# Yongda1/Ab-initio-Flexible-Gaussian-Basis-Neural-Network-Quantum-Monte-Carlo

Hardware: AMD Instinct MI355X
Metric: walker·steps/sec + local-energy evals/sec, N2 14e⁻ 4096 walkers, 1/2/4/8 MI355X (higher is better)
Workload: dtype f32

## Files before the change

ab-initio-flexible-gaussian-basis-neural-network-quantum-monte-carlo_amd/csrc/walker_rev.h:

```cpp
#pragma once
#include "jets.h"
#include "layout.h"
#include "kargs.h"
#include "limdrift.h"
#include "gj.h"
#include "electron.h"

namespace aq {

#ifdef AQ_PHASE_PROF
static __device__ unsigned long long aq_phase_cycles[32];
#define AQ_PH(k)                                                                         \
  do {                                                                                   \
    const unsigned long long t_ = __builtin_readcyclecounter();                          \
    if (lane == 0) atomicAdd(&aq_phase_cycles[(ka.proposal ? 16 : 0) + (k)], t_ - t_ph); \
    t_ph = t_;                                                                           \
  } while (0)
#elif defined(AQ_PHASE_MARK)
#define AQ_PH(k) asm volatile(";AQMARK " #k)
#elif defined(AQ_STOP_AFTER)
#define AQ_PH(k)                                                                     \
  do {                                                                               \
    if constexpr (PROP && (k) == AQ_STOP_AFTER) {                                    \
      if (ka.logabs) ((T*)ka.logabs)[conf * 64 + lane] = sm[lane] + sm[lane + 1024]; \
      return;                                                                        \
    }                                                                                \
  } while (0)
#else
#define AQ_PH(k) \
  do {           \
  } while (0)
#endif

#ifdef AQ_ABLATE
#define AQ_ABL(b) (isprop && (ka.ablate & (b)))
#else
#define AQ_ABL(b) false
#endif

template <typename T> __device__ __forceinline__ T pt_rec(T t) {
  return T(0.70710678118654752) * (T(1) - t * t);
}
template <typename T, int N, int A, bool FWDREG = false>
struct SmemRev {
  static constexpr int D0 = 4 * A;
  static constexpr int DFM = 3 * D0 + 8;
  static constexpr int QM = DFM / 4;
  static constexpr int hl_n = N * D0 + N * 4;
  static constexpr int cmax(int a, int b) { return a > b ? a : b; }
  static constexpr int xs = 0;
  static constexpr int hl = 48;
  static constexpr int hbar = hl;
  static constexpr int QL = (3 * 4 + 8) / 4;
  static constexpr int cq = hl + hl_n;
  static constexpr int sv = cq + (FWDREG ? 0 : N * QM + 2 * N * QL);
  static constexpr int cqo(int l, int i) { return l == 0 ? i * QM : N * QM + ((l - 1) * N + i) * QL; }
  static constexpr int g2 = sv + (FWDREG ? 0 : 3 * N * 4);
  static constexpr int yv = g2 + 3 * 2 * N * 4;
  static constexpr int ybar = yv;
  static constexpr int R = yv + N * N;
  static constexpr int ph = R;
  static constexpr int mx = R + N * N * 2;
  static constexpr int dbar = R;
  static constexpr int R_n = cmax(cmax(4 * N * N, 3 * N * N), 4 + 64 * 12);
  static constexpr int pv = g2;
  static constexpr int RW = (N + 3) / 4;
  static constexpr int st = ((g2 + 3 * N + 2 + 3) / 4) * 4;
  static constexpr int zr = st + (4 * RW * 4 * 4 + (int)sizeof(T) - 1) / (int)sizeof(T);
  static_assert(zr + 4 <= g2 + 3 * 2 * N * 4, "slot table outside the g2 region");
  static constexpr int jdo = R + R_n;
  static constexpr bool hand = FWDREG;
  static constexpr int th = (jdo + (FWDREG ? 64 : 0) + 3) / 4 * 4;
  static constexpr int end = hand ? th + 2 * 2 * 16 * 4 : jdo + (FWDREG ? 64 : 0);
  static constexpr int bytes = ((end * (int)sizeof(T)) + 15) & ~15;
  static constexpr int hoff(int l) { return l == 0 ? 0 : N * D0; }
};

template <int N, int A>
struct WCache {
  static constexpr int D0 = 4 * A;
  static constexpr int yv = 0;
  static constexpr int h0 = yv + N * N;
  static constexpr int loc = h0 + N * D0;
  static constexpr int jaev = loc + (N + D0) * 48;
  static constexpr int jaed = jaev + N;
  static constexpr int g2 = jaed + 48;
  static constexpr int jee = g2 + 3 * 2 * N * 4;
  static constexpr int pv = jee + 1;
  static constexpr int pt = ((pv + 3 * N + 2 + 3) / 4) * 4;
  static constexpr int size = ((pt + 8 * N * N + 63) / 64) * 64;
};
template <int N, int A>
struct ECache {
  static constexpr int D0 = 4 * A;
  static constexpr int yv = 0;
  static constexpr int h0 = N;
  static constexpr int yd = N + D0;
  static constexpr int hd = yd + 3 * N;
  static constexpr int jv = hd + 3 * D0;
  static constexpr int jd = jv + 1;
  static constexpr int xp = jd + 3;
  static constexpr int size = ((xp + 3 + 15) / 16) * 16;
};

template <typename T, int N, int A>
__device__ __forceinline__ void pair_values(const T d[3], cptr<T> P, T out[3][4], T tq[2][4]) {
  using Ly = Lay<N, A>;
  const T RSQ2 = T(0.70710678118654752);
  T p[4];
  p[0] = f_sqrt(d[0] * d[0] + d[1] * d[1] + d[2] * d[2]);
#pragma unroll
  for (int c = 0; c < 3; ++c) p[1 + c] = d[c];
#pragma unroll
  for (int f = 0; f < 4; ++f) out[0][f] = p[f];
#pragma unroll
  for (int j = 0; j < 2; ++j) {
    const cptr<T> dw = P + (j == 0 ? Ly::dbl_w0 : Ly::dbl_w1);
    const cptr<T> db = P + (j == 0 ? Ly::dbl_b0 : Ly::dbl_b1);
    T q[4];
#pragma unroll
    for (int o = 0; o < 4; ++o) {
      T s = db[o];
#pragma unroll
      for (int m = 0; m < 4; ++m) s += p[m] * dw[m * 4 + o];
      q[o] = f_tanh(s);
    }
#pragma unroll
    for (int o = 0; o < 4; ++o) {
      tq[j][o] = q[o];
      p[o] = (p[o] + q[o]) * RSQ2;
      out[j + 1][o] = p[o];
    }
  }
}
template <typename T, int N, int A>
__device__ __forceinline__ void pair_values(const T d[3], cptr<T> P, T out[3][4]) {
  T tq[2][4];
  pair_values<T, N, A>(d, P, out, tq);
}

template <typename T> __device__ __forceinline__ T class4_sum(T x) {
  x += dpp<0x124>(x);
  x += dpp<0x128>(x);
  x += __shfl_xor(x, 16);
  x += __shfl_xor(x, 32);
  return x;
}
template <int M, typename T> __device__ __forceinline__ T quad_bcast(T x) {
  return dpp<M | (M << 2) | (M << 4) | (M << 6)>(x);
}

template <typename T, int NV, int NU>
__device__ __forceinline__ void ld_use(cptr<T> p, T* out) {
  static_assert(NU <= NV, "record");
  if constexpr (sizeof(T) == 4) {
    typedef float f4 __attribute__((ext_vector_type(4)));
// ... 276 lines not shown
    }
#pragma unroll
    for (int o = 0; o < 4; ++o) p1[o] = (p0[o] + f1[o]) * RSQ2;
#pragma unroll
    for (int o = 0; o < 4; ++o) {
      T s = Pq[Ly::dbl_b1 + o];
#pragma unroll
      for (int m = 0; m < 4; ++m) s += p1[m] * Pq[Ly::dbl_w1 + m * 4 + o];
      f2[o] = f_tanh(s);
    }
#pragma unroll
    for (int o = 0; o < 4; ++o) {
      t1[o] = fresh ? pt_rec(f1[o]) : t1[o];
      t2[o] = fresh ? pt_rec(f2[o]) : t2[o];
    }
  }
  T pb2[4], pb1[4], pb0[4];
#pragma unroll
  for (int f = 0; f < 4; ++f) pb2[f] = g2b[((2 * 2 + G) * N + i) * 4 + f];
  T z2[4];
#pragma unroll
  for (int o = 0; o < 4; ++o) z2[o] = pb2[o] * t2[o];
#pragma unroll
  for (int m = 0; m < 4; ++m) {
    T s = g2b[((1 * 2 + G) * N + i) * 4 + m] + pb2[m] * RSQ2;
#pragma unroll
    for (int o = 0; o < 4; ++o) s += z2[o] * Pq[Ly::dbl_w1 + m * 4 + o];
    pb1[m] = s;
  }
  T z1[4];
#pragma unroll
  for (int o = 0; o < 4; ++o) z1[o] = pb1[o] * t1[o];
#pragma unroll
  for (int m = 0; m < 4; ++m) {
    T s = g2b[((0 * 2 + G) * N + i) * 4 + m] + pb1[m] * RSQ2;
#pragma unroll
    for (int o = 0; o < 4; ++o) s += z1[o] * Pq[Ly::dbl_w0 + m * 4 + o];
    pb0[m] = s;
  }
  T rb = pb0[0];
  {
    const T den = al * r + T(1);
    rb += and_zero(k < i, cusp * f_rcp(den * den));
  }
  const T ir = f_rcp(r);
#pragma unroll
  for (int c = 0; c < 3; ++c) dbar[(k * N + i) * 3 + c] = pb0[1 + c] + rb * d[c] * ir;
}

template <typename T, int N>
__device__ __forceinline__ void walker_draws(const __attribute__((address_space(4))) KArgs* kl, int conf, int lane) {
  if (kl->dg1 && lane < N) {
    const uint32_t t = (uint32_t)(conf * N + lane);
    const uint64_t seed = kl->seed, step = kl->step;
    float a[3], b[3], c[4];
    philox_normal3f(seed, step, t, 0u, a);
    philox_normal3f(seed, step, t, 1u, b);
    philox_u4(seed, step, t, 2u, c);
#pragma unroll
    for (int k = 0; k < 3; ++k) {
      ((T*)kl->dg1)[(size_t)t * 3 + k] = (T)a[k];
      ((T*)kl->dg2)[(size_t)t * 3 + k] = (T)b[k];
    }
    ((T*)kl->du)[t] = (T)(c[0] - 5.9604644775390625e-08f);
  }
}

template <typename T, int N, int A, bool PREP = false, bool PROP = false, bool PH = false, bool SPL = false>
__global__ __attribute__((amdgpu_flat_work_group_size(1, 64 * (SPL ? 2 : RevWpb<T, PROP, PREP>::value)))) __attribute__((amdgpu_waves_per_eu(RevWaves<T, N, A, PREP, PROP>::value))) void
k_walker_rev(KArgs ka) {
  static_assert(!PH || PREP, "PH is an adjoint-pass instantiation");
  static_assert(!SPL || (!PROP && !PREP), "SPL is a walker-launch instantiation");
  using Ly = Lay<N, A>;
  constexpr bool fwd_reg = PROP;
  constexpr bool xlane = PROP;
  using SM = SmemRev<T, N, A, fwd_reg>;
  using LCc = LapCache<N, A>;
  static_assert(URecordFits<Ly::total_ext>::value && URecordFits<WCache<N, A>::size>::value &&
                    URecordFits<ECache<N, A>::size>::value && URecordFits<LCc::size>::value &&
                    URecordFits<3 * N>::value && sizeof(PairTab<N>) < (1u << 28),
                "record too large for a 32-bit lane offset");
  constexpr int D0 = SM::D0;
  constexpr int WPB = SPL ? 2 : RevWpb<T, PROP, PREP>::value;
  const cptr<T> P = param_ptr<T>(ka.prm);
  extern __shared__ __attribute__((aligned(16))) unsigned char smem_raw[];
  const int wv = WPB > 1 ? __builtin_amdgcn_readfirstlane((int)(threadIdx.x >> 6)) : 0;
  T* sm = (T*)(smem_raw + (SPL ? 0 : wv) * SM::bytes);
  T* xs = sm + SM::xs;

  const bool isprop = PROP ? true : (ka.proposal != 0);
  const int conf = SPL ? xcd_major(blockIdx.x, gridDim.x) : xcd_major(blockIdx.x, gridDim.x) * WPB + wv;
  if (WPB > 1 && conf >= ka.nconf) return;
  const int lane = WPB > 1 ? (int)(threadIdx.x & 63) : (int)threadIdx.x;
  const int lc = lane >> 4;
  const int er = lane & 15;
  const int le = er < N ? er : N - 1;
  const bool val = (lc == 3);
  const bool live = er < N;
  const bool dir = (lc < 3) && live;
  const int nup = ka.nup;
  const T tstep = (T)ka.tstep;
  const T RSQ2 = T(0.70710678118654752);
  const T ginv0 = T(1) / T(nup), ginv1 = T(1) / T(N - nup);
  const int* rowsrc = ka.rowsrc;
#ifdef AQ_PHASE_PROF
  unsigned long long t_ph = __builtin_readcyclecounter();
#endif

  int pb = conf, pi = -1;
  if (isprop) {
    const int mper = ka.mper ? ka.mper : N, mdiv = ka.mdiv ? ka.mdiv : 1;
    pb = conf / mper;
    pi = (conf - pb * mper) / mdiv;
  }
  const T te_walk = (!PROP && isprop && !ka.xnew) ? taueff_wave<T>(ka.taueff, ka.tacc, 0, ka.tstep, ka.tpart) : T(0);
  if (SPL && wv != 0) {
  } else if (!PREP && !isprop && ka.acc.lpn) {
    const T te1 = taueff_wave<T>(ka.acc.taueff, ka.acc.tacc, 0, ka.acc.tstep, ka.acc.tpart);
    const T te2 = taueff_wave<T>(ka.acc.taueff, ka.acc.tacc, 1, ka.acc.tstep, ka.acc.tpart);
    if (lane < N) {
      T xn[3];
      const bool acc = accept_one<T, N>(ka.acc, (const T*)ka.pos, conf, lane, xn, te1, te2);
#pragma unroll
      for (int c = 0; c < 3; ++c) xs[3 * lane + c] = xn[c];
      if (acc) {
#pragma unroll
        for (int c = 0; c < 3; ++c) ((T*)ka.pos)[(size_t)conf * 3 * N + 3 * lane + c] = xn[c];
        if (ka.acc.count) atomicAdd(&ka.acc.count[conf], 1);
      }
    }
  } else if (!PROP && lane < 3 * N) {
    T x = ((const T*)ka.pos)[(size_t)pb * 3 * N + lane];
    if (isprop && lane / 3 == pi) {
      sm[SM::R + (lane - 3 * pi)] = x;
      if (ka.xnew) {
        x = ((const T*)ka.xnew)[(size_t)conf * 3 + (lane - 3 * pi)];
      } else {
        const T z = ((const T*)ka.gauss1)[(size_t)pb * 3 * N + lane];
        const T ge = ((const T*)ka.pgrad)[(size_t)pb * 3 * N + lane] * te_walk;
        x = x + (ge * tstep + f_sqrt(tstep) * z);
      }
    }
    xs[lane] = x;
  }
  if constexpr (SPL) __syncthreads();
  else if constexpr (!PROP) AQ_SYNC();

  AQ_PH(0);
  using WC = WCache<N, A>;
  using EC = ECache<N, A>;
  const bool reuse = !PREP && PROP;
  const bool wfix = !PREP && !PROP && !isprop && ka.pvok != 0;
  T* Wc = (T*)ka.wcache + (size_t)(reuse ? pb : conf) * WC::size;
  if constexpr (PROP) Wc = ubase(Wc);
  T* Lw = PREP ? (T*)ka.lapcache + (size_t)conf * LCc::size : nullptr;
  const T* Eq = reuse ? (const T*)ka.ecache + (size_t)conf * EC::size : nullptr;
  T* Yv = sm + SM::yv;
  T* g2 = sm + SM::g2;
  T jv = T(0), jd1 = T(0), jve = T(0);
  T jsum_p = T(0);
  T pvr = T(0);
  int rsl = 0;
  T jvp = T(0);
  auto f2_pair_values = [&](T cusp, T al) {
    T* S = sm + SM::R + 4;
    const T* xo = sm + SM::R;
    const int o = lane & 15, part = lane >> 4;
    const int os = o < N ? o : N - 1;
    const T* xp = (part & 1) ? xo : xs + pi * 3;
    T d[3];
#pragma unroll
    for (int c = 0; c < 3; ++c) d[c] = (part < 2) ? xs[os * 3 + c] - xp[c] : xp[c] - xs[os * 3 + c];
    T v[3][4], tq[2][4];
    pair_values<T, N, A>(d, P, v, tq);
    if constexpr (SM::hand) {
      if ((part & 1) == 0 && o < N && o != pi) {
#pragma unroll
        for (int j = 0; j < 2; ++j) {
          T* th = (T*)__builtin_assume_aligned(sm + SM::th + (((part >> 1) * 2 + j) * 16 + o) * 4, 16);
#pragma unroll
          for (int f = 0; f < 4; ++f) th[f] = pt_rec(tq[j][f]);
        }
      }
    }
#pragma unroll
    for (int l = 0; l < 3; ++l)
#pragma unroll
      for (int f = 0; f < 4; ++f) S[lane * 12 + l * 4 + f] = v[l][f];
    if (part < 2 && o < N && o != pi) {
      if constexpr (!PROP) {
        cusp = P[Ly::jee_c + pi * N + o];
        al = P[Ly::jee_a + pi * N + o];
      }
      const T je = f_div(cusp * v[0][0], al * v[0][0] + T(1));
      jvp += part == 0 ? je : -je;
    }
  };
  auto jee_params = [&](T& cusp, T& al) {
    const int os = (lane & 15) < N ? (lane & 15) : N - 1;
    const cptr<T> row = P + pi * N;
    cusp = *uat(row + Ly::jee_c, (unsigned)os);
    al = *uat(row + Ly::jee_a, (unsigned)os);
  };
  if (reuse) {
    lds_dma<T, N * N>(Yv, Wc + WC::yv, lane);
    lds_dma<T, N * D0>(sm + SM::hl, Wc + WC::h0, lane);
    lds_dma<T, 3 * 2 * N * 4>(g2, Wc + WC::g2, lane);
    const T eyv = *uat(Eq + EC::yv, (unsigned)(lane < N ? lane : N - 1));
    const T eh0 = *uat(Eq + EC::h0, (unsigned)(lane < D0 ? lane : D0 - 1));
    const bool mvl = lane < 3 * N && lane / 3 == pi;
    T x0 = T(0), xm = T(0), jc = T(0), ja = T(0);
    if constexpr (PROP) {
      const int l3 = lane < 3 * N ? lane : 3 * N - 1;
      x0 = *uat((const T*)ka.pos + (size_t)pb * 3 * N, (unsigned)l3);
      xm = *uat(Eq + EC::xp, (unsigned)(mvl ? lane - 3 * pi : 0));
      jee_params(jc, ja);
      rsl = *uat(rowsrc, (unsigned)(lane < N ? lane : N - 1));
    }
    {
      if constexpr (PROP) {
        const T* js = (er == pi) ? Eq + EC::jv : Wc + WC::jaev + le;
        jv = and_zero(val && live, *js);
        const T* ds = (le == pi) ? Eq + EC::jd + (lc < 3 ? lc : 0) : Wc + WC::jaed + (lane < 48 ? lane : 47);
        jd1 = and_zero(dir, *ds);
        jve = and_zero(lane == 0, Wc[WC::jee]);
      } else {
        const T a = Wc[WC::jaev + le], b = Eq[EC::jv];
        jv = (val && live) ? ((er == pi) ? b : a) : T(0);
        const T a1 = Wc[WC::jaed + (lane < 48 ? lane : 47)], b1 = Eq[EC::jd + (lc < 3 ? lc : 0)];
        jd1 = dir ? ((le == pi) ? b1 : a1) : T(0);
        const T a2 = Wc[WC::jee];
        jve = lane == 0 ? a2 : T(0);
      }
      pvr = *uat(Wc + WC::pv, (unsigned)(lane < 2 * N + 2 ? lane : 2 * N + 1));
    }
    if constexpr (PROP) {
      if (mvl) sm[SM::R + (lane - 3 * pi)] = x0;
      if (lane < 3 * N) xs[lane] = mvl ? xm : x0;
      AQ_SYNC();
      f2_pair_values(jc, ja);
    }
    asm volatile("s_waitcnt vmcnt(0)" ::: "memory");
    if (lane < N) Yv[pi * N + lane] = eyv;
    if (lane < D0) sm[SM::hl + pi * D0 + lane] = eh0;
  } else if (!SPL || wv == 0) {
    if (wfix) pvr = Wc[WC::pv + (lane < 3 * N + 2 ? lane : 3 * N + 1)];
    ElecOut<T, A> eo;
    electron_stage<T, N, A>(P, xs + le * 3, le, lc, eo);
    T* Wl = Wc + WC::loc + lane;
#pragma unroll
    for (int col = 0; col < N; ++col) {
      PJ<T> sy = P[Ly::wy + col] * eo.yst[0];
#pragma unroll
      for (int m = 1; m < NYW; ++m) sy = sy + P[Ly::wy + m * N + col] * eo.yst[m];
      const PJ<T> yt = eo.env * sy;
      if (!PREP && lane < 48) Wl[col * 48] = yt.d1;
      if (val && live) Yv[er * N + col] = yt.v;
    }
#pragma unroll
    for (int m = 0; m < D0; ++m) {
      if (!PREP && lane < 48) Wl[(N + m) * 48] = eo.hf[m].d1;
      if (val && live) sm[SM::hl + er * D0 + m] = eo.hf[m].v;
    }
    jv = (val && live) ? eo.jae.v : T(0);
    jd1 = dir ? eo.jae.d1 : T(0);
    if (!PREP && !isprop) {
      if (val && live) Wc[WC::jaev + er] = eo.jae.v;
      if (lane < 48) Wc[WC::jaed + lane] = jd1;
    }
  }
  AQ_SYNC();
  if (!PREP && !isprop && (!SPL || wv == 0)) {
    for (int idx = lane; idx < N * N; idx += 64) Wc[WC::yv + idx] = Yv[idx];
    for (int idx = lane; idx < N * D0; idx += 64) Wc[WC::h0 + idx] = sm[SM::hl + idx];
  }

  AQ_PH(1);
  if (reuse && !AQ_ABL(1)) {
    T* S = sm + SM::R + 4;
    if constexpr (!PROP) {
      f2_pair_values(T(0), T(0));
      AQ_SYNC();
    }
    jve += jvp;
    if constexpr (fwd_reg) {
      jsum_p = wave_sum(jv + jve);
      sm[SM::jdo + lane] = jd1;
      jv = jve = jd1 = T(0);
    }
    if (lane < 16) {
      if (lane < N && lane != pi) {
        const int Gp = pi >= nup ? 1 : 0;
        const T gw = Gp ? ginv1 : ginv0;
#pragma unroll
        for (int l = 0; l < 3; ++l)
#pragma unroll
          for (int f = 0; f < 4; ++f)
            g2[((l * 2 + Gp) * N + lane) * 4 + f] +=
                (S[lane * 12 + l * 4 + f] - S[(16 + lane) * 12 + l * 4 + f]) * gw;
      }
    } else if (lane < 40) {
      const int t = lane - 16;
      const int l = t >> 3, G = (t >> 2) & 1, f = t & 3;
      const int k0 = G ? nup : 0, k1 = G ? N : nup;
      T acc = T(0);
#pragma unroll
      for (int k = 0; k < N; ++k) {
        const T dv = S[(32 + k) * 12 + l * 4 + f] - S[(48 + k) * 12 + l * 4 + f];
        acc += (k >= k0 && k < k1 && k != pi) ? dv : T(0);
      }
      g2[((l * 2 + G) * N + pi) * 4 + f] += acc * (G ? ginv1 : ginv0);
    }
  } else if (!reuse && (!SPL || wv == 1)) {
    {
      const int i = lane >> 2, kq = lane & 3;
      const bool icol = i < N;
      const int ii = icol ? i : N - 1;
      T acc[3][2][4];
  #pragma unroll
      for (int l = 0; l < 3; ++l)
  #pragma unroll
        for (int G = 0; G < 2; ++G)
  #pragma unroll
          for (int f = 0; f < 4; ++f) acc[l][G][f] = T(0);
      constexpr int NT = (N + 3) / 4;
      T jcp[NT], jap[NT];
  #pragma unroll
      for (int t = 0; t < NT; ++t) {
        const int kk = kq + 4 * t < N ? kq + 4 * t : N - 1;
        jcp[t] = P[Ly::jee_c + kk * N + ii];
        jap[t] = P[Ly::jee_a + kk * N + ii];
      }
      T dwv[2][16], dbv[2][4];
  #pragma unroll
      for (int j = 0; j < 2; ++j) {
        const cptr<T> dw = P + (j == 0 ? Ly::dbl_w0 : Ly::dbl_w1);
        const cptr<T> db = P + (j == 0 ? Ly::dbl_b0 : Ly::dbl_b1);
  #pragma unroll
        for (int k = 0; k < 16; ++k) dwv[j][k] = dw[k];
  #pragma unroll
        for (int k = 0; k < 4; ++k) dbv[j][k] = db[k];
      }
  #pragma unroll
      for (int t = 0; t < NT; ++t) {
        const int k = kq + 4 * t;
        if (k < N) {
          const bool diag = (k == ii);
          T d[3];
  #pragma unroll
          for (int c = 0; c < 3; ++c) d[c] = xs[ii * 3 + c] - xs[k * 3 + c];
          const T r2 = d[0] * d[0] + d[1] * d[1] + d[2] * d[2];
          const T r = f_sqrt(diag ? T(1) : r2);
          T p[4] = {diag ? T(0) : r, diag ? T(0) : d[0], diag ? T(0) : d[1], diag ? T(0) : d[2]};
          if (icol && k < ii) {
            const T cusp = jcp[t], al = jap[t];
            jve += f_div(cusp * r, al * r + T(1));
          }
          const bool G1 = k >= nup;
  #pragma unroll
          for (int f = 0; f < 4; ++f) {
            acc[0][0][f] += G1 ? T(0) : p[f];
            acc[0][1][f] += G1 ? p[f] : T(0);
          }
  #pragma unroll
          for (int j = 0; j < 2; ++j) {
            T q[4];
  #pragma unroll
            for (int o = 0; o < 4; ++o) {
              T s = dbv[j][o];
  #pragma unroll
              for (int m = 0; m < 4; ++m) s += p[m] * dwv[j][m * 4 + o];
              q[o] = f_tanh(s);
            }
            if (!PREP && !isprop && icol && !diag) {
              T* tp = Wc + WC::pt + (k * N + ii) * 8 + j * 4;
#pragma unroll
              for (int o = 0; o < 4; ++o) tp[o] = pt_rec(q[o]);
            }
            if (PREP && icol) {
              T* tp = Lw + LCc::pt + (k * N + ii) * LCc::pt_n + j * 4;
#pragma unroll
              for (int o = 0; o < 4; ++o) tp[o] = q[o];
            }
  #pragma unroll
            for (int o = 0; o < 4; ++o) {
              p[o] = (p[o] + q[o]) * RSQ2;
              acc[j + 1][0][o] += G1 ? T(0) : p[o];
              acc[j + 1][1][o] += G1 ? p[o] : T(0);
            }
          }
        }
// ... 134 lines not shown
  for (int l = 0; l < 3; ++l) {
    const int d1 = l == 0 ? D0 : NH;
    const int DF = 3 * d1 + 8;
    const int Q = DF / 4;
    const int T4 = d1 / 4;
    if (l + 1 < 3) lw_load(l + 1);
    if constexpr (PROP) {
      if (l == 2) orb_load();
    }
    asm volatile("" ::: "memory");
    T hown[D0 / 4];
    if (l == 0) {
#pragma unroll
      for (int t = 0; t < D0 / 4; ++t) hown[t] = hl[ic * D0 + ff + 4 * t];
    } else {
#pragma unroll
      for (int t = 0; t < D0 / 4; ++t) hown[t] = hreg;
    }
    T gown[2][D0 / 4];
#pragma unroll
    for (int t = 0; t < D0 / 4; ++t) {
      if (t < T4) {
        const T x = ilive ? hown[t] : T(0);
        gown[0][t] = class4_sum(inG1 ? T(0) : x) * ginv0;
        gown[1][t] = class4_sum(inG1 ? x : T(0)) * ginv1;
      }
    }
    T zc[SM::QM];
#pragma unroll
    for (int q = 0; q < SM::QM; ++q) {
      if (q < Q) {
        T F;
        if (q < T4) F = hown[q];
        else if (q < 3 * T4) F = gown[(q - T4) / T4][(q - T4) % T4];
        else F = g2[((l * 2 + (q - 3 * T4)) * N + ic) * 4 + ff];
        T z = F * wcv[l][q];
        asm volatile("" : "+v"(z));
        z += dpp<0xB1>(z);
        z += dpp<0x4E>(z);
        zc[q] = z;
      }
    }
    const int QF = Q / 4;
    T cq[SM::QM];
#pragma unroll
    for (int s4 = 0; s4 < SM::QM / 4; ++s4) {
      if (s4 < QF) {
        const int q0 = 4 * s4;
        T z0 = zc[q0], z1 = zc[q0 + 1], z2 = zc[q0 + 2], z3 = zc[q0 + 3];
        asm volatile("" : "+v"(z0), "+v"(z1), "+v"(z2), "+v"(z3));
        const T zs = (ff & 2) ? ((ff & 1) ? z3 : z2) : ((ff & 1) ? z1 : z0);
        const T c = f_tanh(zs * T(0.25) + wcb[l][s4]);
        if constexpr (fwd_reg) cqr[l][s4] = c;
        else if (ilive) cqv[SM::cqo(l, ic) + q0 + ff] = c;
        cq[q0 + 0] = quad_bcast<0>(c);
        cq[q0 + 1] = quad_bcast<1>(c);
        cq[q0 + 2] = quad_bcast<2>(c);
        cq[q0 + 3] = quad_bcast<3>(c);
      }
    }
#pragma unroll
    for (int q = 0; q < SM::QM; ++q) {
      if (q >= 4 * QF && q < Q) {
        cq[q] = f_tanh(zc[q] * T(0.25) + wcb[l][q]);
        if constexpr (fwd_reg) cqr[l][QF + q - 4 * QF] = cq[q];
        else if (ilive && (q & 3) == ff) cqv[SM::cqo(l, ic) + q] = cq[q];
      }
    }
    T z = wsb[l], z1 = T(0);
#pragma unroll
    for (int q = 0; q < SM::QM; ++q)
      if (q < Q) {
        if (q & 1) z1 += cq[q] * wsw[l][q];
        else z += cq[q] * wsw[l][q];
      }
    z += z1;
    const T sval = f_tanh(z);
    if constexpr (fwd_reg) svr[l] = sval;
    else if (ilive) sv[(l * N + ic) * 4 + ff] = sval;
    const T hin = l == 0 ? hl[ic * D0 + ff] : hreg;
    hreg = (d1 == NH) ? (hin + sval) * RSQ2 : sval;
  }
  }
  if (ilive) hl[SM::hoff(3) + ic * 4 + ff] = hreg;
  AQ_SYNC();
  if ((reuse || wfix) && lane < (wfix ? 3 * N + 2 : 2 * N + 2)) sm[SM::pv + lane] = pvr;
  if constexpr (PROP) {
    const int r = (int)pvr;
    const int src = __shfl(rsl, lane < N ? r : 0);
    if (lane < 4 * SM::RW) {
      const bool ok = lane < N;
      const bool up = r < nup;
      const int h = SM::hl + SM::hoff(3) + src * 4;
      int* stab = (int*)(sm + SM::st) + 4 * lane;
      stab[0] = ok ? SM::yv + r * N : SM::yv;
      stab[1] = (ok && up) ? h : SM::zr;
      stab[2] = (ok && !up) ? h : SM::zr;
      stab[3] = ok ? (up ? 0 : 1) : 2;
    }
    if (lane < 4) sm[SM::zr + lane] = T(0);
    AQ_SYNC();
  }

  AQ_PH(3);
  T* Ph = sm + SM::ph;
  T* Mx = sm + SM::mx;
  const T* H3 = hl + SM::hoff(3);
  for (int idx = PROP ? N * N : lane; idx < N * N; idx += 64) {
    const int r = idx / N, col = idx - r * N;
    const int src = rowsrc[r];
    const int sp = r < nup ? 0 : 1;
    T re = T(0), im = T(0);
#pragma unroll
    for (int f = 0; f < 4; ++f) {
      const T hv = H3[src * 4 + f];
      re += hv * P[Ly::orb_w + ((sp * 4 + f) * N + col) * 2 + 0];
      im += hv * P[Ly::orb_w + ((sp * 4 + f) * N + col) * 2 + 1];
    }
    re += P[Ly::orb_b + (sp * N + col) * 2 + 0];
    im += P[Ly::orb_b + (sp * N + col) * 2 + 1];
    Ph[idx * 2 + 0] = re;
    Ph[idx * 2 + 1] = im;
  }
  if constexpr (!PROP) AQ_SYNC();
  T logdet, phr, phi;
  constexpr bool ybar_reg = PROP;
  V2o a2[(N + 3) / 4];
  if (reuse) {
    bool bad = false;
    logdet = phr = phi = T(0);
    if constexpr (PROP) {
      constexpr int RW = (N + 3) / 4;
      using V2 = typename Pair<T>::type;
      const int cc = lane & 15, rg = lane >> 4;
      const T* rec = sm + SM::pv;
      const int ccl = cc < N ? cc : N - 1;
      const V2* w = ow;
      const V2* bsp = obs;
      const int* stab = (const int*)(sm + SM::st) + 4 * RW * rg;
      if constexpr (phi_mfma) {
        typedef float v4f __attribute__((ext_vector_type(4)));
        const int* sti = (const int*)(sm + SM::st) + 4 * (lane & 15);
        const int fq = lane >> 4;
        const float hu = sm[sti[1] + fq], hd = sm[sti[2] + fq];
        int yo4[RW], fl4[RW];
        v4f pre, pim;
#pragma unroll
        for (int t = 0; t < RW; ++t) {
          yo4[t] = stab[4 * t];
          fl4[t] = stab[4 * t + 3];
          pre[t] = fl4[t] == 1 ? pair_re<T>(bsp[1]) : pair_re<T>(bsp[0]);
          pim[t] = fl4[t] == 1 ? pair_im<T>(bsp[1]) : pair_im<T>(bsp[0]);
        }
        pre = __builtin_amdgcn_mfma_f32_16x16x4f32(hu, owm[0], pre, 0, 0, 0);
        pim = __builtin_amdgcn_mfma_f32_16x16x4f32(hu, owm[1], pim, 0, 0, 0);
        pre = __builtin_amdgcn_mfma_f32_16x16x4f32(hd, owm[2], pre, 0, 0, 0);
        pim = __builtin_amdgcn_mfma_f32_16x16x4f32(hd, owm[3], pim, 0, 0, 0);
#pragma unroll
        for (int t = 0; t < RW; ++t) {
          const bool ok = fl4[t] != 2 && cc < N;
          if (ok) {
            const int e = yo4[t] - SM::yv + cc;
            Ph[e * 2 + 0] = pre[t];
            Ph[e * 2 + 1] = pim[t];
          }
          const T y = ok ? sm[yo4[t] + ccl] : T(0);
          a2[t] = pair_make<T>(pre[t] * y, pim[t] * y);
        }
      } else
#pragma unroll
      for (int t = 0; t < RW; ++t) {
        const int yo = stab[4 * t], hu = stab[4 * t + 1], hd = stab[4 * t + 2], fl = stab[4 * t + 3];
        V2 acc = fl == 1 ? bsp[1] : bsp[0];
#pragma unroll
        for (int f = 0; f < 4; ++f) acc = pair_fma<T>(sm[hu + f], w[f], acc);
#pragma unroll
        for (int f = 0; f < 4; ++f) acc = pair_fma<T>(sm[hd + f], w[4 + f], acc);
        const bool ok = fl != 2 && cc < N;
        if (ok) {
          const int e = yo - SM::yv + cc;
          Ph[e * 2 + 0] = pair_re<T>(acc);
          Ph[e * 2 + 1] = pair_im<T>(acc);
        }
        const T y = ok ? sm[yo + ccl] : T(0);
        a2[t] = pair_make<T>(pair_re<T>(acc) * y, pair_im<T>(acc) * y);
      }
      __builtin_amdgcn_s_setprio(1);
      if (!AQ_ABL(4)) gj_fixed_regs<T, N>(a2, Mx, lane, rec, logdet, phr, phi, bad);
      __builtin_amdgcn_s_setprio(0);
    } else
    if (!AQ_ABL(4)) gj_inverse_fixed<T, N>(Ph, Yv, Mx, lane, sm + SM::pv, logdet, phr, phi, bad);
#ifdef AQ_ABLATE
    if (ka.ablate) bad = false;
#endif
    if (bad) {
#ifdef AQ_PHASE_PROF
      if (lane == 0) atomicAdd(&aq_phase_cycles[15], 1ull);
#endif
#ifdef AQ_PHASE_MARK
      AQ_PH(10);
#endif
      gj_inverse<T, N>(Ph, Yv, Mx, lane, logdet, phr, phi);
      if constexpr (ybar_reg) {
        wave_sync();
        const int cc = lane & 15, rg = lane >> 4;
        const int r = (int)sm[SM::pv + (cc < N ? cc : 0)];
#pragma unroll
        for (int t = 0; t < (N + 3) / 4; ++t) {
          const int c = rg * ((N + 3) / 4) + t;
          const int e = ((c < N ? c : 0) * N + r) * 2;
          a2[t] = pair_make<T>(Mx[e], Mx[e + 1]);
        }
      }
#ifdef AQ_PHASE_MARK
      AQ_PH(11);
#endif
    }
  } else {
    bool bad = true;
    if (wfix) gj_inverse_fixed<T, N>(Ph, Yv, Mx, lane, sm + SM::pv, logdet, phr, phi, bad, Wc + WC::pv, 2 * N + 2);
    if (bad) gj_inverse<T, N>(Ph, Yv, Mx, lane, logdet, phr, phi, (!PREP && !isprop) ? Wc + WC::pv : nullptr);
  }
  if constexpr (!PREP) {
    if (ka.value_only) {
      const T jsum = fwd_reg ? jsum_p : wave_sum(jv + jve);
      const T lpsi = logdet + jsum;
      if (lane == 0) {
        if (ka.logabs) ((T*)ka.logabs)[conf] = lpsi;
        if (ka.phase) ((T*)ka.phase)[conf] = f_atan2(phi, phr);
      }
      if (ka.orb) {
        const T je = wave_sum(jve), ja = wave_sum(jv);
        const T sc = f_exp(je / T(N)) * f_exp(ja / T(N));
        T* O = (T*)ka.orb + (size_t)conf * N * N * 2;
        for (int idx = lane; idx < N * N; idx += 64) {
          const T y = Yv[idx] * sc;
          O[2 * idx] = Ph[2 * idx] * y;
          O[2 * idx + 1] = Ph[2 * idx + 1] * y;
        }
      }
      return;
    }
  }
  AQ_SYNC();
#define BRE(c, s) Mx[((c) * N + (s)) * 2]
#define BIM(c, s) Mx[((c) * N + (s)) * 2 + 1]

  AQ_PH(4);
  T* hbar = sm + SM::hbar;
  T* ybar = sm + SM::ybar;
  constexpr bool q_mfma = PREP && sizeof(T) == 4 && NH == 4;
  if (!q_mfma && lane < 4 * N && !AQ_ABL(8)) {
    const int r = lane >> 2, f = lane & 3;
    const int sp = r < nup ? 0 : 1;
    const cptr<T> wrow = uat(ubase(P + Ly::orb_w), (unsigned)((sp * 4 + f) * N * 2));
    T q = T(0), q1 = T(0);
#pragma unroll
    for (int c = 0; c < N; ++c) {
      const T yv = Yv[r * N + c];
      const T wr = wrow[c * 2] * yv;
      const T wi = wrow[c * 2 + 1] * yv;
      const T qc = PH ? wr * BIM(c, r) + wi * BRE(c, r) : wr * BRE(c, r) - wi * BIM(c, r);
      if (c & 1) q1 += qc;
      else q += qc;
    }
    q += q1;
    hbar[SM::hoff(3) + *uat(rowsrc, (unsigned)r) * 4 + f] = q;
  }
  if constexpr (PREP) {
    for (int idx = lane; idx < 2 * N * N; idx += 64) {
      Lw[LCc::bm + idx] = Mx[idx];
      Lw[LCc::ph + idx] = Ph[idx];
    }
    if constexpr (q_mfma) {
      typedef float v4f __attribute__((ext_vector_type(4)));
      constexpr int NM = (4 * N + 15) / 16, NK = (N + 3) / 4;
      const int kq = lane >> 4, e = lane & 15, fq = lane & 3;
      float bre[NK], bim[NK], wr[2][NK], wi[2][NK];
#pragma unroll
      for (int kk = 0; kk < NK; ++kk) {
        const int c = 4 * kk + kq;
        const bool bok = c < N && e < N;
        const int cl = c < N ? c : N - 1, el = e < N ? e : N - 1;
        bre[kk] = bok ? (float)BRE(cl, el) : 0.f;
        bim[kk] = bok ? (float)BIM(cl, el) : 0.f;
#pragma unroll
        for (int sp = 0; sp < 2; ++sp) {
          const float a = P[Ly::orb_w + ((sp * 4 + fq) * N + cl) * 2], b = P[Ly::orb_w + ((sp * 4 + fq) * N + cl) * 2 + 1];
          wr[sp][kk] = c < N ? a : 0.f;
          wi[sp][kk] = c < N ? b : 0.f;
        }
      }
#pragma unroll
      for (int m = 0; m < NM; ++m) {
        const int r = 4 * m + (e >> 2);
        const bool rok = r < N;
        const bool up = r < nup;
        v4f qre = {0.f, 0.f, 0.f, 0.f}, qim = {0.f, 0.f, 0.f, 0.f};
#pragma unroll
        for (int kk = 0; kk < NK; ++kk) {
          const int c = 4 * kk + kq;
          const float y = (rok && c < N) ? (float)Yv[(rok ? r : 0) * N + (c < N ? c : 0)] : 0.f;
          const float ur = (up ? wr[0][kk] : wr[1][kk]) * y, ui = (up ? wi[0][kk] : wi[1][kk]) * y;
          qre = __builtin_amdgcn_mfma_f32_16x16x4f32(ur, bre[kk], qre, 0, 0, 0);
          qre = __builtin_amdgcn_mfma_f32_16x16x4f32(-ui, bim[kk], qre, 0, 0, 0);
          qim = __builtin_amdgcn_mfma_f32_16x16x4f32(ur, bim[kk], qim, 0, 0, 0);
          qim = __builtin_amdgcn_mfma_f32_16x16x4f32(ui, bre[kk], qim, 0, 0, 0);
        }
// ... 217 lines not shown
            const T* gl = gb + (j + 1) * 2 * N * 4;
            T tv[4];
#pragma unroll
            for (int o = 0; o < 4; ++o) tv[o] = tcur[j * 4 + o];
#pragma unroll
            for (int c = 0; c < NC; ++c) {
              T z1[4], z2[4];
#pragma unroll
              for (int o = 0; o < 4; ++o) {
                T a1 = T(0), a2 = (j == 0) ? p2[c][0] * dw[o] : T(0);
#pragma unroll
                for (int mm = 0; mm < 4; ++mm) {
                  a1 += p1[c][mm] * dw[mm * 4 + o];
                  if (j > 0) a2 += p2[c][mm] * dw[mm * 4 + o];
                }
                z1[o] = a1;
                z2[o] = a2;
              }
#pragma unroll
              for (int o = 0; o < 4; ++o) {
                const T sd1 = T(1) - tv[o] * tv[o];
                const T t1 = sd1 * z1[o];
                const T t2 = sd1 * (z2[o] - T(2) * tv[o] * z1[o] * z1[o]);
                p1[c][o] = (p1[c][o] + t1) * RSQ2;
                p2[c][o] = (p2[c][o] + t2) * RSQ2;
                s1[j][c][o] += m * p1[c][o];
                pcurv += m * gl[o] * p2[c][o];
              }
            }
          }
        }
#pragma unroll
        for (int c = 0; c < NC; ++c) {
          s0[c] += dpp<0xB1>(s0[c]);
          s0[c] += dpp<0x4E>(s0[c]);
#pragma unroll
          for (int j = 0; j < 2; ++j)
#pragma unroll
            for (int f = 0; f < 4; ++f) {
              s1[j][c][f] += dpp<0xB1>(s1[j][c][f]);
              s1[j][c][f] += dpp<0x4E>(s1[j][c][f]);
            }
        }
        if (ilv && kq < NC) {
          const int c = C0 + kq;
          const T cnt = T(k1 - k0 - ((ii >= k0 && ii < k1) ? 1 : 0));
          T* o0 = Lw + LCc::sd + ((G * N + ii) * 3 + c) * 4;
          o0[0] = (NC == 1 || kq == 0) ? s0[0] : s0[NC - 1];
#pragma unroll
          for (int f = 1; f < 4; ++f) o0[f] = (f - 1 == c) ? cnt : T(0);
#pragma unroll
          for (int j = 0; j < 2; ++j) {
            T* oj = Lw + (j + 1) * LCc::layer_n + LCc::sd + ((G * N + ii) * 3 + c) * 4;
#pragma unroll
            for (int f = 0; f < 4; ++f) oj[f] = (NC == 1 || kq == 0) ? s1[j][0][f] : s1[j][NC - 1][f];
          }
        }
      }
    };
    pair_pass(std::integral_constant<int, 0>{}, std::integral_constant<int, 2>{});
    pair_pass(std::integral_constant<int, 2>{}, std::integral_constant<int, 1>{});
    pcurv = T(2) * wave_sum(pcurv);
    const T lpsi = logdet + wave_sum(jv + jve);
    if (lane == 0) {
      Lw[LCc::scal] = pcurv;
      if (ka.logabs) ((T*)ka.logabs)[conf] = lpsi;
      if (ka.phase) ((T*)ka.phase)[conf] = f_atan2(phi, phr);
    }
    return;
  }

  const int c4 = lc < 3 ? lc : 0;
  T lv[N + D0];
  auto lv_load = [&]() {
    const bool mov = reuse && le == pi;
    const T* la = mov ? Eq + EC::yd + c4 * N : Wc + WC::loc + (lane < 48 ? lane : 47);
    const T* lb = mov ? Eq + EC::hd + c4 * D0 : Wc + WC::loc + N * 48 + (lane < 48 ? lane : 47);
    const int st = mov ? 1 : 48;
#pragma unroll
    for (int m = 0; m < N; ++m) lv[m] = la[m * st];
#pragma unroll
    for (int m = 0; m < D0; ++m) lv[N + m] = lb[m * st];
  };
  lv_load();
  AQ_PH(6);
  T* dbar = sm + SM::dbar;
  auto pair_adjoint = [&](int k, int i, bool may_fresh, bool fresh, const T* tcache, T cusp, T al) {
    b3_pair_adjoint<T, N, A>(P, xs, g2b, dbar, nup, k, i, may_fresh, fresh, tcache, cusp, al);
  };
  constexpr int NPR = N * (N - 1);
  if (reuse && !AQ_ABL(32)) {
    constexpr int M = 2 * (N - 1);
    constexpr int NIT = (NPR + 63) / 64;
    T tc[NIT][8], jc[NIT], ja[NIT];
    int pk[NIT], pi2[NIT];
    unsigned prow[NIT];
#pragma unroll
    for (int u = 0; u < NIT; ++u) {
      const unsigned code = uat(&pair_tab<N>.v[pi][0], (unsigned)lane)[64 * u];
      const int k = code & 15, i = (code >> 4) & 15;
      pk[u] = k;
      pi2[u] = i;
      prow[u] = code >> 8;
      jc[u] = *uat(P + Ly::jee_c, prow[u]);
      ja[u] = *uat(P + Ly::jee_a, prow[u]);
    }
#pragma unroll
    for (int u = 0; u < NIT; ++u) {
      const T* tp = uat(Wc + WC::pt, prow[u] * 8);
#pragma unroll
      for (int o = 0; o < 8; ++o) tc[u][o] = tp[o];
    }
    if constexpr (SM::hand) {
      const int hp = pk[0] == pi ? 0 : 1, ho = pk[0] == pi ? pi2[0] : pk[0];
      T hv[8];
#pragma unroll
      for (int j = 0; j < 2; ++j) {
        const T* th = (const T*)__builtin_assume_aligned(sm + SM::th + ((hp * 2 + j) * 16 + ho) * 4, 16);
#pragma unroll
        for (int f = 0; f < 4; ++f) hv[j * 4 + f] = th[f];
      }
#pragma unroll
      for (int o = 0; o < 8; ++o) tc[0][o] = lane < M ? hv[o] : tc[0][o];
    }
#pragma unroll
    for (int u = 0; u < NIT; ++u) {
      const int it = lane + 64 * u;
      if (it < NPR) pair_adjoint(pk[u], pi2[u], false, false, tc[u], jc[u], ja[u]);
    }
  } else if (!reuse) {
    if (!PREP && !isprop && ka.wcache) {
      if constexpr (SPL) __syncthreads();
      __builtin_amdgcn_fence(__ATOMIC_RELEASE, "workgroup");
      __builtin_amdgcn_fence(__ATOMIC_ACQUIRE, "workgroup");
      for (int it = lane; it < NPR; it += SPL ? 128 : 64) {
        const int k = it / (N - 1);
        const int jj = it - k * (N - 1);
        const int i = jj + (jj >= k ? 1 : 0);
        pair_adjoint(k, i, false, false, Wc + WC::pt + (k * N + i) * 8, P[Ly::jee_c + k * N + i], P[Ly::jee_a + k * N + i]);
      }
      if constexpr (SPL) __syncthreads();
    } else {
      for (int it = lane; it < NPR; it += 64) {
        const int k = it / (N - 1);
        const int jj = it - k * (N - 1);
        const int i = jj + (jj >= k ? 1 : 0);
        pair_adjoint(k, i, true, true, nullptr, P[Ly::jee_c + k * N + i], P[Ly::jee_a + k * N + i]);
      }
    }
  }
  AQ_SYNC();

  AQ_PH(7);
  T g = fwd_reg ? sm[SM::jdo + lane] : jd1;
  if (!AQ_ABL(64)) {
    T ga = T(0), gb = T(0), gc = T(0);
#pragma unroll
    for (int k = 0; k < N; ++k) {
      const T dk = dbar[(k * N + le) * 3 + c4] - dbar[(le * N + k) * 3 + c4];
      if (k & 1) ga += (k == le) ? T(0) : dk;
      else g += (k == le) ? T(0) : dk;
    }
#pragma unroll
    for (int col = 0; col < N; ++col) {
      if (col & 1) gc = f_fma(ybar[le * N + col], lv[col], gc);
      else gb = f_fma(ybar[le * N + col], lv[col], gb);
    }
#pragma unroll
    for (int m = 0; m < D0; ++m) {
      if (m & 1) gc = f_fma(hbar[le * D0 + m], lv[N + m], gc);
      else gb = f_fma(hbar[le * D0 + m], lv[N + m], gb);
    }
    g = (g + ga) + (gb + gc);
  }

  AQ_PH(8);
  const T gd = dir ? g : T(0);
  const T sumsq = wave_sum(gd * gd);
  const T lpsi = logdet + (fwd_reg ? jsum_p : wave_sum(jv + jve));
  const auto* kl = late_args();
  if (kl->grad && dir) *uat((T*)kl->grad + (size_t)conf * 3 * N, (unsigned)(3 * le + lc)) = g;
  if (kl->gown && dir && le == pi) *uat((T*)kl->gown + (size_t)conf * 3, (unsigned)lc) = g;
  if (lane == 0) {
    if (kl->logabs) ((T*)kl->logabs)[conf] = lpsi;
    if (kl->phase) ((T*)kl->phase)[conf] = f_atan2(phi, phr);
    if (kl->sumsq) ((T*)kl->sumsq)[conf] = sumsq;
    if (kl->tacc) tacc_add(kl->tacc, isprop ? 1 : 0, conf, (double)sumsq);
  }
  if constexpr (!PREP && !SPL) {
    if (!isprop) walker_draws<T, N>(kl, conf, lane);
  }
  AQ_PH(9);
}

}
```

Measured before the change: 15.16 million.

## Compact proposal-kernel LDS layout and park values in shared memory to cut registers

For the proposal (forward-register) instantiation, the shared-memory layout is repacked: Yv aliases the unused cq/sv region, the pair-value scratch and hand table are sized by N instead of 16, and only 48 jd slots are kept. Live register values (pvr, rsl, the Jastrow sum) are parked in LDS across the long middle section instead of staying in registers, and the lv_load is deferred into the last pair-adjoint iteration. A static_assert checks that 12 workgroups fit per CU, so the aim is higher occupancy and lower register pressure at the cost of extra LDS traffic and reloads.

```diff
diff --git a/ab-initio-flexible-gaussian-basis-neural-network-quantum-monte-carlo_amd/csrc/walker_rev.h b/ab-initio-flexible-gaussian-basis-neural-network-quantum-monte-carlo_amd/csrc/walker_rev.h
--- a/ab-initio-flexible-gaussian-basis-neural-network-quantum-monte-carlo_amd/csrc/walker_rev.h
+++ b/ab-initio-flexible-gaussian-basis-neural-network-quantum-monte-carlo_amd/csrc/walker_rev.h
@@ -55,23 +55,27 @@
   static constexpr int cq = hl + hl_n;
   static constexpr int sv = cq + (FWDREG ? 0 : N * QM + 2 * N * QL);
   static constexpr int cqo(int l, int i) { return l == 0 ? i * QM : N * QM + ((l - 1) * N + i) * QL; }
-  static constexpr int g2 = sv + (FWDREG ? 0 : 3 * N * 4);
-  static constexpr int yv = g2 + 3 * 2 * N * 4;
+  static constexpr int g2 = FWDREG ? cq + N * N : sv + 3 * N * 4;
+  static constexpr int yv = FWDREG ? cq : g2 + 3 * 2 * N * 4;
   static constexpr int ybar = yv;
-  static constexpr int R = yv + N * N;
-  static constexpr int ph = R;
-  static constexpr int mx = R + N * N * 2;
+  static constexpr int R = (FWDREG ? g2 + 3 * 2 * N * 4 : yv + N * N);
   static constexpr int dbar = R;
-  static constexpr int R_n = cmax(cmax(4 * N * N, 3 * N * N), 4 + 64 * 12);
   static constexpr int pv = g2;
   static constexpr int RW = (N + 3) / 4;
   static constexpr int st = ((g2 + 3 * N + 2 + 3) / 4) * 4;
   static constexpr int zr = st + (4 * RW * 4 * 4 + (int)sizeof(T) - 1) / (int)sizeof(T);
   static_assert(zr + 4 <= g2 + 3 * 2 * N * 4, "slot table outside the g2 region");
+  static constexpr int ph = FWDREG ? ((zr + 4 + 3) / 4) * 4 : R;
+  static constexpr int mx = ph + N * N * 2;
+  static constexpr int S_n = FWDREG ? 4 + 4 * N * 12 : 4 + 64 * 12;
+  static constexpr int R_n = cmax(cmax(mx + N * N * 2 - R, 3 * N * N), S_n);
   static constexpr int jdo = R + R_n;
+  static constexpr int js = jdo + 48;
+  static constexpr int prk = hl + N * D0;
+  static_assert(3 * N + 2 <= N * 4, "parked pivot record outside the h^3 rows");
   static constexpr bool hand = FWDREG;
-  static constexpr int th = (jdo + (FWDREG ? 64 : 0) + 3) / 4 * 4;
-  static constexpr int end = hand ? th + 2 * 2 * 16 * 4 : jdo + (FWDREG ? 64 : 0);
+  static constexpr int th = (jdo + (FWDREG ? 48 + 1 : 0) + 3) / 4 * 4;
+  static constexpr int end = hand ? th + 2 * 2 * N * 4 : jdo;
   static constexpr int bytes = ((end * (int)sizeof(T)) + 15) & ~15;
   static constexpr int hoff(int l) { return l == 0 ? 0 : N * D0; }
 };
@@ -514,6 +518,8 @@
                 "record too large for a 32-bit lane offset");
   constexpr int D0 = SM::D0;
   constexpr int WPB = SPL ? 2 : RevWpb<T, PROP, PREP>::value;
+  if constexpr (PROP && sizeof(T) == 4 && N == 14 && A == 2)
+    static_assert(12 * WPB * SM::bytes <= 160 * 1024, "proposal workgroup beyond the 12-per-CU LDS budget");
   const cptr<T> P = param_ptr<T>(ka.prm);
   extern __shared__ __attribute__((aligned(16))) unsigned char smem_raw[];
   const int wv = WPB > 1 ? __builtin_amdgcn_readfirstlane((int)(threadIdx.x >> 6)) : 0;
@@ -590,7 +596,6 @@
   T* Yv = sm + SM::yv;
   T* g2 = sm + SM::g2;
   T jv = T(0), jd1 = T(0), jve = T(0);
-  T jsum_p = T(0);
   T pvr = T(0);
   int rsl = 0;
   T jvp = T(0);
@@ -609,16 +614,17 @@
       if ((part & 1) == 0 && o < N && o != pi) {
 #pragma unroll
         for (int j = 0; j < 2; ++j) {
-          T* th = (T*)__builtin_assume_aligned(sm + SM::th + (((part >> 1) * 2 + j) * 16 + o) * 4, 16);
+          T* th = (T*)__builtin_assume_aligned(sm + SM::th + (((part >> 1) * 2 + j) * N + o) * 4, 16);
 #pragma unroll
           for (int f = 0; f < 4; ++f) th[f] = pt_rec(tq[j][f]);
         }
       }
     }
+    T* Sr = S + (part * N + os) * 12;
 #pragma unroll
     for (int l = 0; l < 3; ++l)
 #pragma unroll
-      for (int f = 0; f < 4; ++f) S[lane * 12 + l * 4 + f] = v[l][f];
+      for (int f = 0; f < 4; ++f) Sr[l * 4 + f] = v[l][f];
     if (part < 2 && o < N && o != pi) {
       if constexpr (!PROP) {
         cusp = P[Ly::jee_c + pi * N + o];
@@ -675,6 +681,10 @@
     asm volatile("s_waitcnt vmcnt(0)" ::: "memory");
     if (lane < N) Yv[pi * N + lane] = eyv;
     if (lane < D0) sm[SM::hl + pi * D0 + lane] = eh0;
+    if constexpr (PROP) {
+      if (lane < 2 * N + 2) sm[SM::prk + lane] = pvr;
+      if (lane < N) ((int*)(sm + SM::prk + 2 * N + 2))[lane] = rsl;
+    }
   } else if (!SPL || wv == 0) {
     if (wfix) pvr = Wc[WC::pv + (lane < 3 * N + 2 ? lane : 3 * N + 1)];
     ElecOut<T, A> eo;
@@ -716,8 +726,8 @@
     }
     jve += jvp;
     if constexpr (fwd_reg) {
-      jsum_p = wave_sum(jv + jve);
-      sm[SM::jdo + lane] = jd1;
+      sm[SM::js] = wave_sum(jv + jve);
+      if (lane < 48) sm[SM::jdo + lane] = jd1;
       jv = jve = jd1 = T(0);
     }
     if (lane < 16) {
@@ -729,7 +739,7 @@
 #pragma unroll
           for (int f = 0; f < 4; ++f)
             g2[((l * 2 + Gp) * N + lane) * 4 + f] +=
-                (S[lane * 12 + l * 4 + f] - S[(16 + lane) * 12 + l * 4 + f]) * gw;
+                (S[lane * 12 + l * 4 + f] - S[(N + lane) * 12 + l * 4 + f]) * gw;
       }
     } else if (lane < 40) {
       const int t = lane - 16;
@@ -738,7 +748,7 @@
       T acc = T(0);
 #pragma unroll
       for (int k = 0; k < N; ++k) {
-        const T dv = S[(32 + k) * 12 + l * 4 + f] - S[(48 + k) * 12 + l * 4 + f];
+        const T dv = S[(2 * N + k) * 12 + l * 4 + f] - S[(3 * N + k) * 12 + l * 4 + f];
         acc += (k >= k0 && k < k1 && k != pi) ? dv : T(0);
       }
       g2[((l * 2 + G) * N + pi) * 4 + f] += acc * (G ? ginv1 : ginv0);
@@ -1039,6 +1049,11 @@
     hreg = (d1 == NH) ? (hin + sval) * RSQ2 : sval;
   }
   }
+  if constexpr (PROP) {
+    pvr = sm[SM::prk + (lane < 2 * N + 2 ? lane : 2 * N + 1)];
+    rsl = ((const int*)(sm + SM::prk + 2 * N + 2))[lane < N ? lane : N - 1];
+    wave_sync();
+  }
   if (ilive) hl[SM::hoff(3) + ic * 4 + ff] = hreg;
   AQ_SYNC();
   if ((reuse || wfix) && lane < (wfix ? 3 * N + 2 : 2 * N + 2)) sm[SM::pv + lane] = pvr;
@@ -1180,7 +1195,7 @@
   }
   if constexpr (!PREP) {
     if (ka.value_only) {
-      const T jsum = fwd_reg ? jsum_p : wave_sum(jv + jve);
+      const T jsum = fwd_reg ? sm[SM::js] : wave_sum(jv + jve);
       const T lpsi = logdet + jsum;
       if (lane == 0) {
         if (ka.logabs) ((T*)ka.logabs)[conf] = lpsi;
@@ -1564,7 +1579,7 @@
 #pragma unroll
     for (int m = 0; m < D0; ++m) lv[N + m] = lb[m * st];
   };
-  lv_load();
+  if constexpr (!PROP) lv_load();
   AQ_PH(6);
   T* dbar = sm + SM::dbar;
   auto pair_adjoint = [&](int k, int i, bool may_fresh, bool fresh, const T* tcache, T cusp, T al) {
@@ -1598,7 +1613,7 @@
       T hv[8];
 #pragma unroll
       for (int j = 0; j < 2; ++j) {
-        const T* th = (const T*)__builtin_assume_aligned(sm + SM::th + ((hp * 2 + j) * 16 + ho) * 4, 16);
+        const T* th = (const T*)__builtin_assume_aligned(sm + SM::th + ((hp * 2 + j) * N + ho) * 4, 16);
 #pragma unroll
         for (int f = 0; f < 4; ++f) hv[j * 4 + f] = th[f];
       }
@@ -1608,6 +1623,9 @@
 #pragma unroll
     for (int u = 0; u < NIT; ++u) {
       const int it = lane + 64 * u;
+      if constexpr (PROP) {
+        if (u == NIT - 1) lv_load();
+      }
       if (it < NPR) pair_adjoint(pk[u], pi2[u], false, false, tc[u], jc[u], ja[u]);
     }
   } else if (!reuse) {
@@ -1634,7 +1652,7 @@
   AQ_SYNC();
 
   AQ_PH(7);
-  T g = fwd_reg ? sm[SM::jdo + lane] : jd1;
+  T g = fwd_reg ? sm[SM::jdo + (lane < 48 ? lane : 47)] : jd1;
   if (!AQ_ABL(64)) {
     T ga = T(0), gb = T(0), gc = T(0);
 #pragma unroll
@@ -1659,7 +1677,7 @@
   AQ_PH(8);
   const T gd = dir ? g : T(0);
   const T sumsq = wave_sum(gd * gd);
-  const T lpsi = logdet + (fwd_reg ? jsum_p : wave_sum(jv + jve));
+  const T lpsi = logdet + (fwd_reg ? sm[SM::js] : wave_sum(jv + jve));
   const auto* kl = late_args();
   if (kl->grad && dir) *uat((T*)kl->grad + (size_t)conf * 3 * N, (unsigned)(3 * le + lc)) = g;
   if (kl->gown && dir && le == pi) *uat((T*)kl->gown + (size_t)conf * 3, (unsigned)lc) = g;
```

After: 15.26 million, median of 6. Within noise of the previous version (+0.7%).
